# wienkers/marEx

Hardware: AMD Instinct MI355X
Metric: Mcells*timesteps/s, shifting_baseline + hobday_extreme p95 (validation+anomaly+thresholds+mask) (higher is better)
Workload: dtype f32

## Files before the change

### marex_amd/csrc/marex_tails.hip

```cpp
#include "marex_common.hip.h"
#include "marex_tails.hip.h"

typedef __amdgpu_buffer_rsrc_t tl_rsrc_t;
__device__ __forceinline__ tl_rsrc_t tl_make_rsrc(const void* base) {
    return __builtin_amdgcn_make_buffer_rsrc(const_cast<void*>(base), 0, -1, 0x00020000);
}
__device__ __forceinline__ uint4 tl_load_chunk(tl_rsrc_t r, unsigned voff, unsigned soff) {
    typedef unsigned u4 __attribute__((ext_vector_type(4)));
    const u4 v = __builtin_amdgcn_raw_buffer_load_b128(r, (int)voff, (int)soff, 0);
    return make_uint4(v.x, v.y, v.z, v.w);
}
__device__ __forceinline__ unsigned pk_sub_sat_u16(unsigned a, unsigned b) {
    unsigned r;
    asm("v_pk_sub_u16 %0, %1, %2 clamp" : "=v"(r) : "v"(a), "v"(b));
    return r;
}
__device__ __forceinline__ unsigned pk_add_u16(unsigned a, unsigned b) {
    unsigned r;
    asm("v_pk_add_u16 %0, %1, %2" : "=v"(r) : "v"(a), "v"(b));
    return r;
}
__device__ __forceinline__ unsigned pk_sub_u16(unsigned a, unsigned b) {
    unsigned r;
    asm("v_pk_sub_u16 %0, %1, %2" : "=v"(r) : "v"(a), "v"(b));
// ... 100 lines not shown
                }
                {
                    float mx = -__builtin_inff();
#pragma unroll
                    for (int u = 0; u < 16; ++u) mx = fmaxf(mx, fmaxf(va[u], vb[u]));
                    if (__builtin_amdgcn_ballot_w64(mx >= e_last) != 0) {
                        unsigned sa = ovf & 0xFFFFu, sb = ovf >> 16;
#pragma unroll
                        for (int u = 0; u < 16; ++u) {
                            if (va[u] >= e_last) sa = tail_ovf_add(sa, (unsigned)(r + u));
                            if (vb[u] >= e_last) sb = tail_ovf_add(sb, (unsigned)(r + u));
                        }
                        ovf = sa | (sb << 16);
                    }
                }
                sort16_desc(half[hb]);
            }
            unsigned v[32];
            if (short_list) {
#pragma unroll
                for (int i = 0; i < 16; ++i) {
                    v[i] = half[0][i];
                    v[16 + i] = 0u;
                }
            } else {
#pragma unroll
                for (int i = 0; i < 16; ++i) {
                    v[i] = half[0][i];
                    v[16 + i] = half[1][15 - i];
                }
                bitonic_merge_desc<32>(v);
            }
            if (active) {
#pragma unroll
                for (int j = 0; j < 4; ++j) {
                    if (j >= nch) break;
                    uint4 w0, w1;
                    unsigned* a = reinterpret_cast<unsigned*>(&w0);
                    unsigned* b = reinterpret_cast<unsigned*>(&w1);
#pragma unroll
                    for (int i = 0; i < 4; ++i) {
                        const unsigned x = v[8 * j + 2 * i], y = v[8 * j + 2 * i + 1];
                        a[i] = (x & 0xFFFFu) | (y << 16);
                        b[i] = (x >> 16) | (y & 0xFFFF0000u);
                    }
                    lists[(((size_t)d0 * NPER + p) * nch + j) * C + c] = w0;
                    lists[(((size_t)d1 * NPER + p) * nch + j) * C + c] = w1;
                }
            }
        }
        if (active) {
            aux[(size_t)d0 * C + c] = tail_aux_word(cnt & 0xFFFFu, ovf & 0xFFFFu);
            aux[(size_t)d1 * C + c] = tail_aux_word(cnt >> 16, ovf >> 16);
        }
    }
    };
    if (lean)
        body(std::true_type{});
    else
        body(std::false_type{});
}

static bool tails_geometry(int max_bucket, int list_rows, int& nper, int& nch) {
    if (max_bucket < 1 || max_bucket > TAIL_MAX_BUCKET || list_rows < 8 || list_rows > 32) return false;
    nper = (max_bucket + list_rows - 1) / list_rows;
    nch = list_rows <= 16 ? 2 : 4;
    return true;
}

extern "C" int marex_tail_lists(int max_bucket, int list_rows) {
    int nper, nch;
    return tails_geometry(max_bucket, list_rows, nper, nch) ? nper : -1;
}

int marex_tail_extract_impl(marex_ctx* ctx, const float* anom, int64_t T_out, int64_t C, const int32_t* doy_start,
                            const int32_t* doy_rows, int max_bucket, const float* edges, int nb, int list_rows, void* lists,
                            uint32_t* aux, const int* skip_chunks) {
    if (!ctx) return -1;
    if (!anom || !doy_start || !doy_rows || !edges || !lists || !aux || T_out <= 0 || C <= 0)
        return fail(ctx, -1, "marex_tail_extract_f32: null pointer or empty shape");
    if (nb < 4 || nb > TAIL_MAX_NB) return fail(ctx, -4, "marex_tail_extract_f32: nb must be in 4..%d", TAIL_MAX_NB);
    int nper, nch;
    if (!tails_geometry(max_bucket, list_rows, nper, nch))
        return fail(ctx, -4, "marex_tail_extract_f32: dayofyear buckets must hold 1..%d rows, lists 8..32 rows", TAIL_MAX_BUCKET);
    if (((uintptr_t)lists & 15) != 0) return fail(ctx, -1, "marex_tail_extract_f32: lists must be 16-byte aligned");
    if (C * 4 > 0xFFFFFFFFll) return fail(ctx, -4, "marex_tail_extract_f32: more than 2^30 cells");
    HIP_TRY(ctx, hipSetDevice(ctx->device));
    const size_t need = (size_t)T_out * sizeof(long long);
    if (need > ctx->row_off_bytes) {
        if (ctx->row_off) HIP_TRY(ctx, hipFree(ctx->row_off));
        ctx->row_off = nullptr;
        ctx->row_off_bytes = 0;
        HIP_TRY(ctx, hipMalloc((void**)&ctx->row_off, need));
        ctx->row_off_bytes = need;
    }
    const unsigned ncb = (unsigned)((C + 255) / 256);
    unsigned chunks = (2048 + ncb - 1) / ncb;
    chunks = chunks < 1 ? 1 : (chunks > 61 ? 61 : chunks);
    const size_t lds = (size_t)(nb + 1) * sizeof(float);
    {
        LaunchTimer lt(ctx, MAREX_K_TAILS);
        hipLaunchKernelGGL(k_row_offsets, dim3((unsigned)((T_out + 255) / 256)), dim3(256), 0, ctx->stream, doy_rows, (long)T_out, (long)C,
                           ctx->row_off, (int)sizeof(float));
        hipLaunchKernelGGL(k_tail_extract, dim3(ncb, chunks), dim3(256), lds, ctx->stream, anom, (long)C, doy_start, ctx->row_off, edges,
                           nb, nper, list_rows, reinterpret_cast<uint4*>(lists), aux, skip_chunks);
    }
    HIP_TRY(ctx, hipGetLastError());
    return 0;
}

extern "C" int marex_tail_extract_f32(marex_ctx* ctx, const float* anom, int64_t T_out, int64_t C, const int32_t* doy_start,
                                      const int32_t* doy_rows, int max_bucket, const float* edges, int nb, int list_rows,
                                      void* lists, uint32_t* aux) {
    return marex_tail_extract_impl(ctx, anom, T_out, C, doy_start, doy_rows, max_bucket, edges, nb, list_rows, lists, aux, nullptr);
}


#define MAREX_BUMP_KEY(u, w, ext)                                                                                   \
    "v_cmpx_lt_u32_e32 vcc, " #u ", %[n]\n\ts_cbranch_execz 1f\n\t" ext "\n\t"                                      \
    "v_subrev_u32_e32 %[t], %[b0], %[t]\n\tv_min_i32_e32 %[t], %[hi], %[t]\n\tv_and_b32_e32 %[a], -2, %[t]\n\t"       \
    "v_and_b32_e32 %[t], 1, %[t]\n\tv_lshl_add_u32 %[a], %[a], 1, %[col]\n\t"
#define MAREX_BUMP_LO(w) "v_bfe_u32 %[t], %[" #w "], 7, 9"
#define MAREX_BUMP_HI(w) "v_lshrrev_b32_e32 %[t], 23, %[" #w "]"
template <int SGN>
__device__ __forceinline__ void tl_bump_chunk(const uint4& ch, int n, int B0, int BWp1, unsigned col_lds) {
    unsigned t, a;
    unsigned long long sv;
    const int mul = SGN > 0 ? 65535 : -65535;
#define MAREX_BUMP_ADD(one) "v_mad_i32_i24 %[t], %[t], %[mul], " one "\n\tds_add_u32 %[a], %[t]\n\t"
#define MAREX_BUMP_ALL(one)                                                                                          \
    "s_mov_b64 %[sv], exec\n\t"                                                                                      \
    MAREX_BUMP_KEY(0, x, MAREX_BUMP_LO(x)) MAREX_BUMP_ADD(one) MAREX_BUMP_KEY(1, x, MAREX_BUMP_HI(x)) MAREX_BUMP_ADD(one)   \
    MAREX_BUMP_KEY(2, y, MAREX_BUMP_LO(y)) MAREX_BUMP_ADD(one) MAREX_BUMP_KEY(3, y, MAREX_BUMP_HI(y)) MAREX_BUMP_ADD(one)   \
    MAREX_BUMP_KEY(4, z, MAREX_BUMP_LO(z)) MAREX_BUMP_ADD(one) MAREX_BUMP_KEY(5, z, MAREX_BUMP_HI(z)) MAREX_BUMP_ADD(one)   \
    MAREX_BUMP_KEY(6, w, MAREX_BUMP_LO(w)) MAREX_BUMP_ADD(one) MAREX_BUMP_KEY(7, w, MAREX_BUMP_HI(w)) MAREX_BUMP_ADD(one)   \
    "1:\n\ts_mov_b64 exec, %[sv]"
    if (SGN > 0)
        asm volatile(MAREX_BUMP_ALL("1")
                     : [t] "=&v"(t), [a] "=&v"(a), [sv] "=&s"(sv)
                     : [n] "v"(n), [x] "v"(ch.x), [y] "v"(ch.y), [z] "v"(ch.z), [w] "v"(ch.w), [b0] "s"(B0), [hi] "s"(BWp1), [col] "v"(col_lds), [mul] "s"(mul)
                     : "vcc", "memory");
    else
        asm volatile(MAREX_BUMP_ALL("-1")
                     : [t] "=&v"(t), [a] "=&v"(a), [sv] "=&s"(sv)
                     : [n] "v"(n), [x] "v"(ch.x), [y] "v"(ch.y), [z] "v"(ch.z), [w] "v"(ch.w), [b0] "s"(B0), [hi] "s"(BWp1), [col] "v"(col_lds), [mul] "s"(mul)
                     : "vcc", "memory");
#undef MAREX_BUMP_ALL
#undef MAREX_BUMP_ADD
}
#undef MAREX_BUMP_KEY
#undef MAREX_BUMP_LO
#undef MAREX_BUMP_HI

#define TT_LS 34
#ifndef TT_BW
#define TT_BW 64
#endif
#define TT_MARGIN 6
#ifndef TT_STEP
#define TT_STEP 56
#endif
static_assert(TT_STEP <= TT_BW - 8, "straggler passes must overlap: a quantile bin between two tried bands would never be found");
#define TT_NPF 2

template <int NPERT>
struct TailBucket {
    uint4 c0[NPERT < TT_NPF ? NPERT : TT_NPF];
    unsigned aux;
    int d;
};

template <int P, int TC, int NT, int NPERT, int TR_ = NT / TC>
__global__ void __launch_bounds__(NT, NT == 256 ? 4 : (NT == 512 ? 2 : 1))
k_thr_tails(const uint4* __restrict__ lists, const unsigned* __restrict__ aux, int NPER, int nch, const float* __restrict__ anom,
            long C, int ny, int nx, int row0, int row1, int tiles_x, int Dd, const float* __restrict__ centres, int nb, double q,
            int wd, float lower_bound, float upper_bound, float* __restrict__ thr, marex_thr_stats* __restrict__ stats,
            unsigned long long* __restrict__ dbg, int pass_limit) {
    constexpr int TR = TR_;
    constexpr int NCELL = TR * TC;
    constexpr int NPF = NPERT < TT_NPF ? NPERT : TT_NPF;
    static_assert(NCELL <= NT && NT - NCELL < 64, "tile does not match the thread count");
    constexpr int OR = TR - 2 * P, OC = TC - 2 * P;
    __shared__ unsigned lev[NT * TT_LS];
    __shared__ unsigned tot_s[NT];
    __shared__ int s_lo[2], s_hi[2];
    __shared__ int s_iumin[2], s_iumax[2];
    __shared__ int s_est_min, s_est_max;

    const int t = threadIdx.x;
    const bool spare = NCELL < NT && t >= NCELL;
    const int tc = t % TC;
    const int tr = (TR > 1) ? (t / TC + P) % TR : 0;
    const int ci = spare ? t : tr * TC + tc;
    const int ty = (int)blockIdx.x / tiles_x, tx = (int)blockIdx.x - ty * tiles_x;
    const int jt0 = row0 + ty * OR, it0 = tx * OC;
    const int j = (ny > 0) ? jt0 - P + tr : 0;
    const int icol = it0 - P + tc;
    bool cell_valid;
    long cell;
    if (ny > 0) {
        int gi = icol % nx;
        if (gi < 0) gi += nx;
        cell_valid = (j >= 0 && j < ny) && !spare;
        cell = (long)j * nx + gi;
    } else {
        cell_valid = icol < nx && !spare;
        cell = icol < nx ? icol : nx - 1;
    }
    if (!cell_valid) cell = 0;
    const bool is_out = !spare && tr >= P && tr < TR - P && tc >= P && tc < TC - P && j < row1 && icol < nx && (ny > 0 ? j >= row0 : true);
    const int d_begin = (int)blockIdx.y * Dd;
    const int ndays = (NDOY - d_begin) < Dd ? (NDOY - d_begin) : Dd;
    const int pd = wd / 2;
    bool land = true;
    if (is_out) land = !(anom[cell] == anom[cell]);
    if (!__syncthreads_or(is_out && !land)) {
        if (is_out)
            for (int dd = 0; dd < ndays; ++dd) thr[(size_t)(d_begin + dd) * C + cell] = nan_f();
        return;
    }
    if (is_out && land)
        for (int dd = 0; dd < ndays; ++dd) thr[(size_t)(d_begin + dd) * C + cell] = nan_f();

    unsigned* mycol = &lev[ci * TT_LS];
    uint2* mycol2 = reinterpret_cast<uint2*>(mycol);
    typedef __attribute__((address_space(3))) unsigned lds_u32;
    const unsigned col_lds = (unsigned)(size_t)(lds_u32*)mycol;
    const int base_max = nb - TT_BW > 0 ? nb - TT_BW : 0;
    auto clamp_base = [&](int b) { return b < 0 ? 0 : (b > base_max ? base_max : b); };
    int B0 = 0;
    int BW = nb < TT_BW ? nb : TT_BW;
    constexpr int NLP = (TT_BW + 2 + 1) / 2;
    const unsigned voff = (unsigned)cell * 16u;
    const unsigned chunk_row = (unsigned)C * 16u;
    const size_t day_stride = (size_t)NPER * nch * (size_t)C;

    auto load_bucket = [&](int d0) {
        TailBucket<NPERT> b;
        b.d = d0;
        const tl_rsrc_t r = tl_make_rsrc(lists + (size_t)d0 * day_stride);
#pragma unroll
        for (int p = 0; p < NPF; ++p)
            b.c0[p] = (p < NPER) ? tl_load_chunk(r, voff, (unsigned)(nch * p) * chunk_row) : make_uint4(0, 0, 0, 0);
        b.aux = aux[(size_t)d0 * C + cell];
        return b;
    };
    auto bump = [&](int k, int sgn) {
        const int odd = k & 1;
        unsigned addr;
        asm("v_lshl_add_u32 %0, %1, 1, %2" : "=v"(addr) : "v"(k - odd), "v"(col_lds));
        int v;
        const int mul = sgn > 0 ? 65535 : -65535, one = sgn > 0 ? 1 : -1;
        asm("v_mad_i32_i24 %0, %1, %2, %3" : "=v"(v) : "v"(odd), "v"(mul), "v"(one));
        __hip_atomic_fetch_add((lds_u32*)(size_t)addr, (unsigned)v, __ATOMIC_RELAXED, __HIP_MEMORY_SCOPE_WORKGROUP);
    };
    int mytot = 0;
    constexpr bool ctx_asm_bump = true;
    auto bump_chunk = [&](const uint4& ch, int n, int sgn, int nfix) {
#pragma unroll
        for (int u = 0; u < 8; ++u) {
            const bool on = n > u;
            if (u >= nfix && __builtin_amdgcn_ballot_w64(on) == 0) break;
            if (on) {
                int lvl = tl_bin1(ch, u) - B0;
                lvl = lvl > BW + 1 ? BW + 1 : lvl;
                bump(lvl, sgn);
            }
        }
    };
    auto apply_bucket = [&](const TailBucket<NPERT>& b, int sgn) {
        const int cnt = cell_valid ? (int)(b.aux & 0x3FFu) : 0;
        const unsigned lim = ((unsigned)(B0 + 1) << TAIL_POS_BITS) - 1u;
        const unsigned lim_rep = lim | (lim << 16);
        const tl_rsrc_t r = tl_make_rsrc(lists + (size_t)b.d * day_stride);
        int n_in = 0;
        auto one_list = [&](const uint4& ch, int p) {
            const int n = cnt > 0 ? tl_count_above(ch, lim_rep) : 0;
            n_in += n;
            if (ctx_asm_bump) { if (sgn > 0) tl_bump_chunk<1>(ch, n, B0, BW + 1, col_lds); else tl_bump_chunk<-1>(ch, n, B0, BW + 1, col_lds); }
            else bump_chunk(ch, n, sgn, NPERT >= 3 ? 2 : 1);
            bool full = n == 8;
#pragma unroll
            for (int jj = 1; jj < 4; ++jj) {
                if (jj >= nch || __builtin_amdgcn_ballot_w64(full) == 0) break;
                const uint4 cj = tl_load_chunk(r, voff, (unsigned)(nch * p + jj) * chunk_row);
                const int nj = full ? tl_count_above(cj, lim_rep) : 0;
                n_in += nj;
                if (ctx_asm_bump) { if (sgn > 0) tl_bump_chunk<1>(cj, nj, B0, BW + 1, col_lds); else tl_bump_chunk<-1>(cj, nj, B0, BW + 1, col_lds); }
                else bump_chunk(cj, nj, sgn, 0);
                full = nj == 8;
            }
        };
#pragma unroll
        for (int p = 0; p < NPF; ++p)
            if (p < NPER) one_list(b.c0[p], p);
#pragma nounroll
        for (int p = NPF; p < NPER; p += 2) {
            const uint4 e0 = tl_load_chunk(r, voff, (unsigned)(nch * p) * chunk_row);
            const uint4 e1 = p + 1 < NPER ? tl_load_chunk(r, voff, (unsigned)(nch * (p + 1)) * chunk_row) : make_uint4(0, 0, 0, 0);
            one_list(e0, p);
            if (p + 1 < NPER) one_list(e1, p + 1);
        }
        const int below = cnt - n_in;
        if (below > 0) __hip_atomic_fetch_add((lds_u32*)(size_t)col_lds, (unsigned)(sgn > 0 ? below : -below), __ATOMIC_RELAXED,
                                              __HIP_MEMORY_SCOPE_WORKGROUP);
        mytot += sgn > 0 ? cnt : -cnt;
    };
    auto prefix = [&]() -> unsigned {
        unsigned run_rep = 0;
#pragma unroll
        for (int i = 0; i < (NLP + 1) / 2; ++i) {
            uint2 w = mycol2[i];
            w.x = pk_add_u16(w.x + (w.x << 16), run_rep);
            run_rep = __builtin_amdgcn_perm(w.x, w.x, 0x03020302u);
            w.y = pk_add_u16(w.y + (w.y << 16), run_rep);
            run_rep = __builtin_amdgcn_perm(w.y, w.y, 0x03020302u);
            mycol2[i] = w;
        }
        return run_rep & 0xFFFFu;
    };
    auto unprefix = [&]() {
        unsigned prev = 0;
#pragma unroll
        for (int i = 0; i < (NLP + 1) / 2; ++i) {
            const uint2 w = mycol2[i];
            uint2 o;
            o.x = pk_sub_u16(w.x, __builtin_amdgcn_alignbit(w.x, prev, 16));
            o.y = pk_sub_u16(w.y, __builtin_amdgcn_alignbit(w.y, w.x, 16));
            prev = w.y;
            mycol2[i] = o;
        }
    };
    auto wrap = [&](int d) { return ((d % NDOY) + NDOY) % NDOY; };
    auto rebuild = [&](int d) {
        for (int r = 0; r < TT_LS / 2; ++r) mycol2[r] = make_uint2(0u, 0u);
        mytot = 0;
        TailBucket<NPERT> cur = load_bucket(wrap(d - pd));
        for (int o = -pd + 1; o <= pd; ++o) {
            const TailBucket<NPERT> nxt = load_bucket(wrap(d + o));
            apply_bucket(cur, +1);
            cur = nxt;
        }
        apply_bucket(cur, +1);
    };
    auto pooled = [&](int k) {
        const unsigned* base = mycol + (k >> 1);
        const int sh16 = (k & 1) * 16;
        int sum = 0;
#pragma unroll
        for (int dr = -P; dr <= P; ++dr)
#pragma unroll
            for (int dc = -P; dc <= P; ++dc) sum += (int)((base[(dr * TC + dc) * TT_LS] >> sh16) & 0xFFFFu);
        return sum;
    };
    auto pooled_tot = [&]() {
        const unsigned* base = &tot_s[tr * TC + tc];
        int sum = 0;
#pragma unroll
        for (int dr = -P; dr <= P; ++dr)
#pragma unroll
            for (int dc = -P; dc <= P; ++dc) sum += (int)base[dr * TC + dc];
        return sum;
    };
    auto window = [&](int start, int (&Wv)[8]) {
        const unsigned* base = mycol + (start >> 1);
        unsigned a0 = 0, a1 = 0, a2 = 0, a3 = 0;
#pragma unroll
        for (int dr = -P; dr <= P; ++dr)
#pragma unroll
            for (int dc = -P; dc <= P; ++dc) {
                const uint2* p2 = reinterpret_cast<const uint2*>(base + (dr * TC + dc) * TT_LS);
                const uint2 u = p2[0], v = p2[1];
                a0 += u.x;
                a1 += u.y;
                a2 += v.x;
                a3 += v.y;
            }
        Wv[0] = (int)(a0 & 0xFFFFu);
        Wv[1] = (int)(a0 >> 16);
        Wv[2] = (int)(a1 & 0xFFFFu);
        Wv[3] = (int)(a1 >> 16);
        Wv[4] = (int)(a2 & 0xFFFFu);
        Wv[5] = (int)(a2 >> 16);
        Wv[6] = (int)(a3 & 0xFFFFu);
        Wv[7] = (int)(a3 >> 16);
    };
    auto find_level = [&](int hint, int khi, double qpos, int& ck, int& cb) {
        const int qf = (int)floor(qpos);
        int top = (khi - 1) & ~3;
        if (top > 60) top = 60;
        if (top < 0) top = 0;
        int start = ((hint >= 0 ? hint : (khi >> 1)) - 2) & ~3;
        start = start < 0 ? 0 : (start > top ? top : start);
        ck = 0;
        cb = 0;
        for (;;) {
            int Wv[8];
            window(start, Wv);
            const int m = (khi - start) < 8 ? (khi - start) : 8;
            int n = 0;
#pragma unroll
            for (int i = 0; i < 8; ++i) n += (i < m) && (Wv[i] <= qf);
            if (n == 0) {
                if (start == 0) {
                    ck = Wv[0];
                    return 0;
                }
                start -= 4;
                continue;
            }
            if (n == m) {
                if (m < 8 || start >= top) {
                    cb = Wv[m - 1];
                    return khi;
                }
                start += 4;
                continue;
            }
            cb = 0;
#pragma unroll
            for (int i = 0; i < 8; ++i) {
                if (i == n - 1) cb = Wv[i];
                if (i == n) ck = Wv[i];
            }
            return start + n;
        }
    };
    unsigned kmin = 0xFFFFFFFFu, kmax = 0u, nlow = 0u, nhigh = 0u;
    auto emit_threshold = [&](int d, int iu, int ck, int cb, double qpos) {
        const int il = iu > 0 ? iu - 1 : 0;
        const int cs_iu = ck;
        const int cs_il = iu > 0 ? cb : ck;
        const int diff = cs_iu - cs_il;
        const double frac = diff > 0 ? (qpos - (double)cs_il) / (double)diff : 0.5;
        const float dc = centres[iu] - centres[il];
        const double prod = frac * (double)dc;
        float t32 = (float)((double)centres[il] + prod);
        if (iu == 0) t32 = centres[0];
        const unsigned key = ordered_key(t32);
        kmin = key < kmin ? key : kmin;
        kmax = key > kmax ? key : kmax;
        if (t32 > upper_bound) ++nhigh;
        if (t32 < lower_bound) {
            ++nlow;
            t32 = lower_bound;
        }
        thr[(size_t)d * C + cell] = t32;
    };

    if (t == 0) {
        s_est_min = 0x7fffffff;
        s_est_max = -1;
        s_lo[0] = s_lo[1] = s_hi[0] = s_hi[1] = 0;
        s_iumin[0] = s_iumin[1] = 0x7fffffff;
        s_iumax[0] = s_iumax[1] = -1;
    }
    __syncthreads();
    {
        const TailBucket<NPERT> b = load_bucket(d_begin);
        const int cnt = cell_valid ? (int)(b.aux & 0x3FFu) : 0;
        if (cnt > 0) {
            int rank = (int)ceil((1.0 - q) * (double)cnt / (double)NPER);
            rank = rank < 1 ? 1 : (rank > 8 ? 8 : rank);
            unsigned key = 0;
#pragma unroll
            for (int u = 0; u < 8; ++u)
                if (u == rank - 1) key = tl_key(b.c0[0], u);
            if (key != 0u) {
                const int est = (int)(key >> TAIL_POS_BITS) - 1;
                atomicMin(&s_est_min, est);
                atomicMax(&s_est_max, est);
            }
        }
    }
    __syncthreads();
    {
        const int emin = s_est_min, emax = s_est_max;
        if (emax >= 0) {
            const int span = emax - emin + 1;
            B0 = clamp_base(span <= TT_BW - 2 * TT_MARGIN ? emin - (TT_BW - span) / 2 : emin - TT_MARGIN);
        }
    }
    BW = nb - B0 < TT_BW ? nb - B0 : TT_BW;

    int hint = -1;
    bool need_rebuild = true;
    unsigned long long n_rebuild = 0, n_pass = 0;
    TailBucket<NPERT> pin, pout;
    pin.d = pout.d = 0;
    pin.aux = pout.aux = 0;
#pragma unroll
    for (int p = 0; p < NPF; ++p) pin.c0[p] = pout.c0[p] = make_uint4(0, 0, 0, 0);
#ifdef MAREX_STAMPS
    unsigned long long st_p1 = 0, st_p2 = 0, st_bar = 0;
#define STAMP() __builtin_amdgcn_s_memtime()
#endif
    for (int dd = 0; dd < ndays; ++dd) {
        const int d = d_begin + dd;
        const int dpar = dd & 1;
#ifdef MAREX_STAMPS
        const unsigned long long tA = STAMP();
#endif
        if (need_rebuild) {
            rebuild(d);
            need_rebuild = false;
            ++n_rebuild;
            hint = -1;
        } else {
            unprefix();
            apply_bucket(pin, +1);
            apply_bucket(pout, -1);
        }
        tot_s[ci] = prefix();
        if (dd + 1 < ndays) {
            pin = load_bucket(wrap(d + 1 + pd));
            pout = load_bucket(wrap(d - pd));
        }
#ifdef MAREX_STAMPS
        const unsigned long long tB = STAMP();
        st_p1 += tB - tA;
#endif
        bool resolved = !(is_out && !land);
        int tried_lo = B0, tried_hi = B0;
        bool excursion = false;
        for (int pass = 0;; ++pass) {
            const int par = pass & 1;
#ifdef MAREX_STAMPS
            const unsigned long long tC0 = STAMP();
#endif
            __syncthreads();
#ifdef MAREX_STAMPS
            const unsigned long long tC = STAMP();
            st_bar += tC - tC0;
#endif
            if (t == 0) {
                s_lo[par ^ 1] = 0;
                s_hi[par ^ 1] = 0;
                if (pass == 0) {
                    s_iumin[dpar ^ 1] = 0x7fffffff;
                    s_iumax[dpar ^ 1] = -1;
                }
            }
            int iu_lo = 0x7fffffff, iu_hi = -1;
            if (!resolved) {
                const int tot = pooled_tot();
                if (tot > 0) {
                    const double qpos = q * (double)tot;
                    int ck, cb;
                    int k = find_level(hint, BW + 1, qpos, ck, cb);
                    int iu = -1;
                    if (k >= 1 && k <= BW) {
                        iu = B0 + k - 1;
                        hint = k;
                    } else if (k > BW && B0 + BW >= nb) {
                        iu = nb - 1;
                        k = iu - B0 + 1;
                        ck = pooled(k);
                        cb = pooled(k - 1);
                        hint = k;
                    } else if (k > BW) {
                        atomicOr(&s_hi[par], 1);
                        hint = -1;
                    } else {
                        atomicOr(&s_lo[par], 1);
                        hint = -1;
                    }
                    if (iu >= 0) {
                        emit_threshold(d, iu, ck, cb, qpos);
                        iu_lo = iu_hi = iu;
                        resolved = true;
                    }
                } else {
                    thr[(size_t)d * C + cell] = nan_f();
                    resolved = true;
                }
            }
            if (__builtin_amdgcn_ballot_w64(iu_hi >= 0) != 0) {
                const int wlo = wave_min_i32(iu_lo), whi = wave_max_i32(iu_hi);
                if ((t & 63) == 0) {
                    atomicMin(&s_iumin[dpar], wlo);
                    atomicMax(&s_iumax[dpar], whi);
                }
            }
#ifdef MAREX_STAMPS
            const unsigned long long tD = STAMP();
            st_p2 += tD - tC;
#endif
            __syncthreads();
#ifdef MAREX_STAMPS
            st_bar += STAMP() - tD;
#endif
            const int lo = s_lo[par], hi = s_hi[par];
            if (!lo && !hi) break;
            if (pass >= pass_limit) {
                if (!resolved) {
                    thr[(size_t)d * C + cell] = nan_f();
                    atomicAdd(&stats->n_unresolved, 1u);
                }
                break;
            }
            if (lo) {
                B0 = clamp_base(tried_lo - TT_STEP);
                tried_lo = B0;
            } else {
                B0 = clamp_base(tried_hi + TT_STEP);
                tried_hi = B0;
            }
            BW = nb - B0 < TT_BW ? nb - B0 : TT_BW;
            excursion = true;
            rebuild(d);
            tot_s[ci] = prefix();
            hint = -1;
            ++n_pass;
        }
        if (dd + 1 < ndays) {
            const int imin = s_iumin[dpar], imax = s_iumax[dpar];
            if (imax >= 0) {
                const int span = imax - imin + 1;
                const bool near_edge = imin - B0 < TT_MARGIN || (B0 + BW - 1) - imax < TT_MARGIN;
                if (excursion || near_edge) {
                    const int want = clamp_base(span <= TT_BW - 2 * TT_MARGIN ? imin - (TT_BW - span) / 2 : imin - TT_MARGIN);
                    if (want != B0) {
                        B0 = want;
                        BW = nb - B0 < TT_BW ? nb - B0 : TT_BW;
                        need_rebuild = true;
                    }
                }
            }
        }
    }
    for (int sft = 32; sft > 0; sft >>= 1) {
        const unsigned a = __shfl_down(kmin, sft, 64), b = __shfl_down(kmax, sft, 64);
        kmin = a < kmin ? a : kmin;
        kmax = b > kmax ? b : kmax;
        nlow += __shfl_down(nlow, sft, 64);
        nhigh += __shfl_down(nhigh, sft, 64);
    }
    if ((t & 63) == 0) {
        if (kmin != 0xFFFFFFFFu) atomicMin(&stats->min_key, kmin);
        if (kmax != 0u) atomicMax(&stats->max_key, kmax);
        if (nlow) atomicAdd(&stats->n_too_low, nlow);
        if (nhigh) atomicAdd(&stats->n_too_high, nhigh);
    }
#ifdef MAREX_STAMPS
#ifdef MAREX_STAMPS_WAVE
    const int st_wave = MAREX_STAMPS_WAVE >= 0 ? MAREX_STAMPS_WAVE : (int)((blockIdx.x + blockIdx.y) % (NT / 64));
    if (dbg && t == st_wave * 64) {
#else
    if (dbg && t == 0) {
#endif
        atomicAdd(&dbg[5], st_p1);
        atomicAdd(&dbg[6], st_p2);
        atomicAdd(&dbg[7], st_bar);
    }
#endif
    if (dbg && t == 0) {
        atomicAdd(&dbg[0], n_rebuild);
        atomicAdd(&dbg[2], n_pass);
        atomicAdd(&dbg[3], (unsigned long long)ndays);
    }
}

template <int NSC>
__global__ void __launch_bounds__(64)
k_thr_cells(const uint4* __restrict__ lists, const unsigned* __restrict__ aux, int NPER, int nch, const float* __restrict__ anom,
            long C, long c0, long c1, int nblk, const float* __restrict__ centres, int nb, double q, int wd, float lower_bound,
            float upper_bound, float* __restrict__ thr, marex_thr_stats* __restrict__ stats, unsigned long long* __restrict__ dbg) {
// ... 114 lines not shown
                        n = ne;
                        exact = true;
                        f = (double)(tot - n) <= qpos;
                        ++n_exact;
                    }
                }
                if (go) {
                    if (f) {
                        lo = mid;
                        n_lo = n;
                        lo_exact = exact;
                    } else {
                        hi = mid;
                        n_hi = n;
                    }
                }
            }
            const int iu = hi;
            if (__builtin_amdgcn_ballot_w64(iu > 0 && !lo_exact) != 0) {
                const int ne = count_exact(d, iu);
                if (iu > 0 && !lo_exact) {
                    n_lo = ne;
                    ++n_exact;
                }
            }
            const int il = iu > 0 ? iu - 1 : 0;
            const int cs_iu = tot - n_hi, cs_il = iu > 0 ? tot - n_lo : cs_iu;
            const int diff = cs_iu - cs_il;
            const double frac = diff > 0 ? (qpos - (double)cs_il) / (double)diff : 0.5;
            const float dc = centres[iu] - centres[il];
            const double prod = frac * (double)dc;
            t32 = (float)((double)centres[il] + prod);
            if (iu == 0) t32 = centres[0];
            if (valid && !land) {
                const unsigned key = ordered_key(t32);
                kmin = key < kmin ? key : kmin;
                kmax = key > kmax ? key : kmax;
                if (t32 > upper_bound) ++nhigh;
                if (t32 < lower_bound) ++nlow;
            }
            if (t32 < lower_bound) t32 = lower_bound;
        }
        if (valid) thr[(size_t)d * C + cell] = land ? nan_f() : t32;
    }
    for (int sft = 32; sft > 0; sft >>= 1) {
        const unsigned a = __shfl_down(kmin, sft, 64), b = __shfl_down(kmax, sft, 64);
        kmin = a < kmin ? a : kmin;
        kmax = b > kmax ? b : kmax;
        nlow += __shfl_down(nlow, sft, 64);
        nhigh += __shfl_down(nhigh, sft, 64);
        n_exact += __shfl_down(n_exact, sft, 64);
    }
    if (lane == 0) {
        if (kmin != 0xFFFFFFFFu) atomicMin(&stats->min_key, kmin);
        if (kmax != 0u) atomicMax(&stats->max_key, kmax);
        if (nlow) atomicAdd(&stats->n_too_low, nlow);
        if (nhigh) atomicAdd(&stats->n_too_high, nhigh);
        if (dbg && n_exact) atomicAdd(&dbg[1], n_exact);
    }
}

extern "C" int marex_hobday_thresholds_tails_f32(marex_ctx* ctx, const void* lists, const uint32_t* aux, int list_rows,
                                                 const float* anom, int64_t T_out, int64_t C, int ny, int nx, int max_bucket,
                                                 const float* centres,
                                                 int nb, double q, int wd, int ws, float lower_bound, float upper_bound, int row0,
                                                 int row1, float* thr_doy_major, marex_thr_stats* stats) {
    if (!ctx) return -1;
    if (!lists || !aux || !anom || !centres || !thr_doy_major || !stats || T_out <= 0 || C <= 0)
        return fail(ctx, -1, "marex_hobday_thresholds_tails_f32: null pointer or empty shape");
    if (wd < 3 || wd > 365 || (wd & 1) == 0)
        return fail(ctx, -1, "marex_hobday_thresholds_tails_f32: window_days_hobday must be odd and in 3..365");
    if (ws < 1 || (ws & 1) == 0) return fail(ctx, -1, "marex_hobday_thresholds_tails_f32: window_spatial_hobday must be odd");
    if (!(q > 0.0 && q <= 1.0)) return fail(ctx, -1, "marex_hobday_thresholds_tails_f32: q must be in (0, 1]");
    if (ny == 0) {
        if (ws > 1) return fail(ctx, -1, "marex_hobday_thresholds_tails_f32: spatial pooling needs a structured grid");
        nx = (int)C;
        row0 = 0;
        row1 = 1;
    } else if ((int64_t)ny * nx != C) {
        return fail(ctx, -1, "marex_hobday_thresholds_tails_f32: ny*nx != C");
    } else if (row0 < 0 || row1 > ny || row0 >= row1) {
        return fail(ctx, -1, "marex_hobday_thresholds_tails_f32: need 0 <= row0 < row1 <= ny");
    }
    const int p = ws / 2;
    if (nb < 4 || nb > TAIL_MAX_NB || max_bucket < 1 || max_bucket > TAIL_MAX_BUCKET || p > 3 ||
        (int64_t)max_bucket * wd * ws * ws > 65535 || C > (1 << 24))
        return fail(ctx, -4, "marex_hobday_thresholds_tails_f32: shape outside the tail kernel (nb <= %d, buckets <= %d rows, "
                             "ws <= 7, pooled window <= 65535 samples)", TAIL_MAX_NB, TAIL_MAX_BUCKET);
    HIP_TRY(ctx, hipSetDevice(ctx->device));
    int NPER, nch;
    if (!tails_geometry(max_bucket, list_rows, NPER, nch))
        return fail(ctx, -4, "marex_hobday_thresholds_tails_f32: %d rows per bucket in lists of %d", max_bucket, list_rows);
    const int cells_opt = ctx_opt(ctx, "THR_CELLS", 1);
    if (p == 0 && cells_opt && (cells_opt == 2 ? wd * NPER <= 128 : wd * NPER <= 16)) {
        const long c0 = ny > 0 ? (long)row0 * nx : 0, c1 = ny > 0 ? (long)row1 * nx : (long)C;
        const long ncg = (c1 - c0 + 63) / 64;
        int nblk = (int)((32L * 4 * device_cus(ctx) + ncg - 1) / ncg);
        nblk = nblk < 1 ? 1 : (nblk > 12 ? 12 : nblk);
        nblk = ctx_opt(ctx, "THR_CELLS_BLOCKS", nblk);
        LaunchTimer lt(ctx, MAREX_K_THRESHOLDS);
        const size_t lds = (size_t)((wd * NPER + 3) & ~3) * 64 * sizeof(uint4);
        const int nslot = (wd * NPER + 3) & ~3;
        const bool cached = nslot == 12 && ctx_opt(ctx, "THR_CELLS_CACHE", 1);
        if (lds > 64 * 1024) HIP_TRY(ctx, hipFuncSetAttribute((const void*)k_thr_cells<0>, hipFuncAttributeMaxDynamicSharedMemorySize, (int)lds));
        hipLaunchKernelGGL(cached ? k_thr_cells<12> : k_thr_cells<0>, dim3((unsigned)ncg, (unsigned)nblk), dim3(64), lds, ctx->stream,
                           reinterpret_cast<const uint4*>(lists), aux, NPER, nch, anom, (long)C, c0, c1, nblk, centres, nb, q, wd,
                           lower_bound, upper_bound, thr_doy_major, stats, ctx_debug_counters(ctx));
        HIP_TRY(ctx, hipGetLastError());
        return 0;
    }
    if (NPER > 6)
        return fail(ctx, -4, "marex_hobday_thresholds_tails_f32: %d rows per bucket in lists of %d: more than 6 lists", max_bucket, list_rows);
    const int tile_pref = ctx_opt(ctx, "THR_TILE", (ny > 0 && p > 0 && max_bucket >= 24) ? 32 : 16);
    const bool half = (ny > 0 && p == 2) && tile_pref == 3216 && (row1 - row0) >= 12 && nx >= 16;
    const bool big = !half && (ny > 0 && p > 0) && tile_pref == 32 && (row1 - row0) >= 16 && nx >= 16;
    const int NT = big ? 1024 : (half ? 512 : 256);
    int TR = (ny > 0 && p > 0) ? (big ? 32 : 16) : 1, TC = NT / TR;
    const size_t lds_pad = (size_t)ctx_opt(ctx, "THR_LDS_PAD", 0) * 1024;
    bool tall = false;
    if (big && p == 2 && ctx_opt(ctx, "THR_TALL", 1)) {
        auto ntiles = [&](int tr, int tc) {
            return (long)((nx + tc - 2 * p - 1) / (tc - 2 * p)) * ((row1 - row0 + tr - 2 * p - 1) / (tr - 2 * p));
        };
        tall = ntiles(34, 30) < ntiles(32, 32) && (row1 - row0) >= 30;
        if (tall) TR = 34, TC = 30;
    }
    const int OR = TR - 2 * p, OC = TC - 2 * p;
    const int tiles_x = (nx + OC - 1) / OC, tiles_y = (row1 - row0 + OR - 1) / OR;
    int Dd = ctx_opt(ctx, "THR_DD", 0);
    if (Dd < 1 || Dd > NDOY) {
        const long cus = device_cus(ctx), tiles = (long)tiles_x * tiles_y;
        const long slots = cus * (big ? 1 : (half ? 2 : 4));
        long best = -1;
        for (int d = 16; d <= NDOY; ++d) {
            const long blocks = tiles * ((NDOY + d - 1) / d);
            const long cost = ((blocks + slots - 1) / slots) * (d + wd);
            if (best < 0 || cost < best) best = cost, Dd = d;
        }
    }
    dim3 grid((unsigned)(tiles_x * tiles_y), (unsigned)((NDOY + Dd - 1) / Dd));
    unsigned long long* dbg = ctx_debug_counters(ctx);
    const uint4* tl = reinterpret_cast<const uint4*>(lists);
    const int pass_limit = ctx_opt(ctx, "THR_PASS_LIMIT", 2 * (nb / TT_STEP) + 9);
#define MAREX_TT_ARGS tl, aux, NPER, nch, anom, (long)C, ny, nx, row0, row1, tiles_x, Dd, centres, nb, q, wd, lower_bound, upper_bound, thr_doy_major, stats, dbg, pass_limit
#define MAREX_TT_LAUNCH(PP, TCC, NTT, ...)                                                                                           \
    do {                                                                                                                             \
        if (NPER <= 1)                                                                                                               \
            hipLaunchKernelGGL((k_thr_tails<PP, TCC, NTT, 1, ##__VA_ARGS__>), grid, dim3(NTT), lds_pad, ctx->stream, MAREX_TT_ARGS); \
        else if (NPER <= 2)                                                                                                          \
            hipLaunchKernelGGL((k_thr_tails<PP, TCC, NTT, 2, ##__VA_ARGS__>), grid, dim3(NTT), lds_pad, ctx->stream, MAREX_TT_ARGS); \
        else                                                  \
            hipLaunchKernelGGL((k_thr_tails<PP, TCC, NTT, 3, ##__VA_ARGS__>), grid, dim3(NTT), lds_pad, ctx->stream, MAREX_TT_ARGS); \
    } while (0)
    {
        LaunchTimer lt(ctx, MAREX_K_THRESHOLDS);
        if (TR == 1)
            MAREX_TT_LAUNCH(0, 256, 256);
        else if (half)
            MAREX_TT_LAUNCH(2, 32, 512, 16);
        else if (big && p == 1)
            MAREX_TT_LAUNCH(1, 32, 1024);
        else if (big && p == 2 && tall)
            MAREX_TT_LAUNCH(2, 30, 1024, 34);
        else if (big && p == 2)
            MAREX_TT_LAUNCH(2, 32, 1024);
        else if (big)
            MAREX_TT_LAUNCH(3, 32, 1024);
        else if (p == 1)
            MAREX_TT_LAUNCH(1, 16, 256);
        else if (p == 2)
            MAREX_TT_LAUNCH(2, 16, 256);
        else
            MAREX_TT_LAUNCH(3, 16, 256);
    }
#undef MAREX_TT_LAUNCH
#undef MAREX_TT_ARGS
    HIP_TRY(ctx, hipGetLastError());
    return 0;
}

#ifndef MASK_WAVES
#define MASK_WAVES 5
#endif
template <int NPERT>
__global__ void __launch_bounds__(256, MASK_WAVES)
k_mask_tails(const uint4* __restrict__ lists, const unsigned* __restrict__ aux, int NPER_all, int nch, const float* __restrict__ anom,
             const float* __restrict__ edges, int nb, const float* __restrict__ thr, const int* __restrict__ doy_start,
             const int* __restrict__ doy_rows, const long long* __restrict__ row_off, const long long* __restrict__ row_off_anom,
             long C, long c0, long c1, unsigned char* __restrict__ out, unsigned long long* __restrict__ n_true,
             unsigned long long* __restrict__ dbg) {
    const int nchunk = (int)gridDim.y;
    const int dA = (int)blockIdx.y * NDOY / nchunk, dB = ((int)blockIdx.y + 1) * NDOY / nchunk;
    const long c = (c0 & ~255L) + ((long)blockIdx.x * 256 + threadIdx.x) * 4;
    unsigned cnt_true = 0;
    unsigned long long n_slow = 0;
    if (c >= c0 && c < c1) {
        const float inv_width = (float)(nb - 1) / (edges[nb] - edges[1]);
        for (int d = dA; d < dB; ++d) {
            const int r0 = doy_start[d], nd = doy_start[d + 1] - r0;
            if (nd == 0) continue;
            const float4 th4 = *reinterpret_cast<const float4*>(thr + (size_t)d * C + c);
            const float tv[4] = {th4.x, th4.y, th4.z, th4.w};
            const uint4 ax = *reinterpret_cast<const uint4*>(aux + (size_t)d * C + c);
            const unsigned av[4] = {ax.x, ax.y, ax.z, ax.w};
            unsigned beyond = 0;
            unsigned bits[4][4];
            unsigned lim_ge[4];
            int kt[4];
            bool slow = false, walk[4];
#pragma unroll
            for (int i = 0; i < 4; ++i) {
                bits[i][0] = bits[i][1] = bits[i][2] = bits[i][3] = 0u;
                const bool isnum = tv[i] == tv[i];
                kt[i] = isnum ? digitize_bin(tv[i], edges, nb, inv_width) : nb;
                slow = slow || (isnum && (av[i] & TAIL_AUX_BEYOND) && ((av[i] & TAIL_AUX_MANY) || kt[i] >= nb));
                beyond |= (isnum && (av[i] & TAIL_AUX_BEYOND)) ? 1u : 0u;
                walk[i] = isnum && (av[i] & 0x3FFu) > 0 && kt[i] < nb;
                const unsigned lim = ((unsigned)(kt[i] + 1) << TAIL_POS_BITS) - 1u;
                lim_ge[i] = lim | (lim << 16);
            }
            auto set_prefix = [&](const uint4& q, int n, int i) {
#pragma unroll
                for (int u = 0; u < 8; ++u) {
                    const bool on = n > u;
                    if (u >= 1 && __builtin_amdgcn_ballot_w64(on) == 0) break;
                    if (on) {
                        const int pos = (int)(tl_key(q, u) & (TAIL_MAX_BUCKET - 1));
#pragma unroll
                        for (int wi = 0; wi < 4; ++wi)
                            if ((pos >> 5) == wi) bits[i][wi] |= 1u << (pos & 31);
                    }
                }
            };
            if (__builtin_amdgcn_ballot_w64(!slow) != 0)
            for (int pg = 0; pg < NPER_all; pg += NPERT) {
                const int NPER = (NPER_all - pg) < NPERT ? (NPER_all - pg) : NPERT;
                uint4 ch[NPERT][4];
                const uint4* row0 = lists + (((size_t)d * NPER_all + pg) * nch) * C + c;
#pragma unroll
                for (int p = 0; p < NPERT; ++p)
#pragma unroll
                    for (int i = 0; i < 4; ++i) ch[p][i] = p < NPER ? row0[(size_t)(p * nch) * C + i] : make_uint4(0, 0, 0, 0);
            float cand_val[NPERT][4];
            int cand_pos[NPERT][4];
            unsigned redo = 0;
            {
#pragma unroll
                for (int p = 0; p < NPERT; ++p) {
#pragma unroll
                    for (int i = 0; i < 4; ++i) {
                        cand_pos[p][i] = -1;
                        cand_val[p][i] = 0.f;
                        if (p < NPER && walk[i] && !slow) {
                            const unsigned lgt = lim_ge[i] + (0x10001u << TAIL_POS_BITS);
                            const int n_ge = tl_count_above(ch[p][i], lim_ge[i]);
                            const int n_gt = tl_count_above(ch[p][i], lgt);
                            set_prefix(ch[p][i], n_gt, i);
                            if (n_ge == 8 || n_ge - n_gt > 1) redo |= 1u << (p * 4 + i);
                            if (n_ge - n_gt == 1) {
                                const unsigned w[4] = {ch[p][i].x, ch[p][i].y, ch[p][i].z, ch[p][i].w};
                                unsigned lo = w[0], hi = w[1];
#pragma unroll
                                for (int k = 1; k < 4; ++k)
                                    if ((n_gt >> 1) == k) lo = w[k], hi = k < 3 ? w[k + 1] : 0u;
                                const unsigned key = (n_gt & 1) ? (lo >> 16) : (lo & 0xFFFFu);
                                (void)hi;
                                cand_pos[p][i] = (int)(key & (TAIL_MAX_BUCKET - 1));
                            }
                        }
                    }
                }
#pragma unroll
                for (int p = 0; p < NPERT; ++p)
#pragma unroll
                    for (int i = 0; i < 4; ++i)
                        if (cand_pos[p][i] >= 0)
                            cand_val[p][i] = *reinterpret_cast<const float*>(reinterpret_cast<const char*>(anom) + row_off_anom[r0 + cand_pos[p][i]] + (size_t)(c + i) * 4);
#pragma unroll
                for (int p = 0; p < NPERT; ++p)
#pragma unroll
                    for (int i = 0; i < 4; ++i)
                        if (cand_pos[p][i] >= 0 && cand_val[p][i] >= tv[i]) {
                            const int pos = cand_pos[p][i];
#pragma unroll
                            for (int wi = 0; wi < 4; ++wi)
                                if ((pos >> 5) == wi) bits[i][wi] |= 1u << (pos & 31);
                        }
                if (__builtin_amdgcn_ballot_w64(redo != 0u) != 0) {
#pragma unroll
                    for (int p = 0; p < NPERT; ++p)
#pragma unroll
                        for (int i = 0; i < 4; ++i) {
                            if (__builtin_amdgcn_ballot_w64((redo >> (p * 4 + i)) & 1u) == 0) continue;
                            bool on = (redo >> (p * 4 + i)) & 1u;
                            for (int jj = 0; jj < nch; ++jj) {
                                if (__builtin_amdgcn_ballot_w64(on) == 0) break;
                                const uint4 q = on ? row0[(size_t)(p * nch + jj) * C + i] : make_uint4(0, 0, 0, 0);
#pragma unroll
                                for (int u = 0; u < 8; ++u) {
                                    const unsigned key = tl_key(q, u);
                                    const int bin = (int)(key >> TAIL_POS_BITS) - 1, pos = (int)(key & (TAIL_MAX_BUCKET - 1));
                                    on = on && bin >= kt[i];
                                    if (on) {
                                        bool ext = bin > kt[i];
                                        if (!ext) ext = *reinterpret_cast<const float*>(reinterpret_cast<const char*>(anom) + row_off_anom[r0 + pos] + (size_t)(c + i) * 4) >= tv[i];
                                        if (ext) {
#pragma unroll
                                            for (int wi = 0; wi < 4; ++wi)
                                                if ((pos >> 5) == wi) bits[i][wi] |= 1u << (pos & 31);
// ... 133 lines not shown
```

Before: 309,700.

## Add lean tail-threshold kernel specialization with fused inline-asm list scan

Adds a compile-time specialized 'lean' variant of the thresholds kernel for the common geometry (six lists, two chunks each, big tiles, p=2). It fixes NPER and nch as template constants, replaces per-list count-then-bump with a single inline-asm scan that compares, bumps LDS counters and propagates a 'full' wave mask in one pass, and walks day pointers incrementally instead of recomputing wrapped offsets. The goal is to cut VALU instructions, ballots and address arithmetic in the per-day sliding-window update. The cost is extra template instantiations and hand-written asm that only fires on this exact geometry, selected through an option that defaults to on.

```diff
diff --git a/marex_amd/csrc/marex_tails.hip b/marex_amd/csrc/marex_tails.hip
--- a/marex_amd/csrc/marex_tails.hip
+++ b/marex_amd/csrc/marex_tails.hip
@@ -276,6 +276,46 @@
 #undef MAREX_BUMP_LO
 #undef MAREX_BUMP_HI
 
+#define MAREX_SCAN_KEY(ext)                                                                                           \
+    ext "\n\tv_cmpx_lt_u32_e32 vcc, %[b0], %[t]\n\ts_cbranch_execz 1f\n\t"
+#define MAREX_SCAN_ADD(one)                                                                                           \
+    "v_subrev_u32_e32 %[t], %[b0], %[t]\n\tv_min_i32_e32 %[t], %[hi], %[t]\n\tv_and_b32_e32 %[a], -2, %[t]\n\t"         \
+    "v_and_b32_e32 %[t], 1, %[t]\n\tv_lshl_add_u32 %[a], %[a], 1, %[col]\n\tv_mad_i32_i24 %[t], %[t], %[mul], " one "\n\t" \
+    "ds_add_u32 %[a], %[t]\n\tv_add_u32_e32 %[n], 1, %[n]\n\t"
+#define MAREX_SCAN_LO(w) "v_bfe_u32 %[t], %[" #w "], 7, 9"
+#define MAREX_SCAN_HI(w) "v_lshrrev_b32_e32 %[t], 23, %[" #w "]"
+template <int SGN>
+__device__ __forceinline__ unsigned long long tl_scan_chunk(const uint4& ch, unsigned long long pm, int& n, int B0, int BWp1,
+                                                            unsigned col_lds) {
+    unsigned t, a;
+    unsigned long long sv, full;
+    const int mul = SGN > 0 ? 65535 : -65535;
+#define MAREX_SCAN_ALL(one)                                                                                           \
+    "s_mov_b64 %[sv], exec\n\ts_mov_b64 %[full], 0\n\ts_and_b64 exec, exec, %[pm]\n\ts_cbranch_execz 1f\n\t"          \
+    MAREX_SCAN_KEY(MAREX_SCAN_LO(x)) MAREX_SCAN_ADD(one) MAREX_SCAN_KEY(MAREX_SCAN_HI(x)) MAREX_SCAN_ADD(one)         \
+    MAREX_SCAN_KEY(MAREX_SCAN_LO(y)) MAREX_SCAN_ADD(one) MAREX_SCAN_KEY(MAREX_SCAN_HI(y)) MAREX_SCAN_ADD(one)         \
+    MAREX_SCAN_KEY(MAREX_SCAN_LO(z)) MAREX_SCAN_ADD(one) MAREX_SCAN_KEY(MAREX_SCAN_HI(z)) MAREX_SCAN_ADD(one)         \
+    MAREX_SCAN_KEY(MAREX_SCAN_LO(w)) MAREX_SCAN_ADD(one) MAREX_SCAN_KEY(MAREX_SCAN_HI(w))                             \
+    "s_mov_b64 %[full], exec\n\t" MAREX_SCAN_ADD(one)                                                                \
+    "1:\n\ts_mov_b64 exec, %[sv]"
+    if (SGN > 0)
+        asm volatile(MAREX_SCAN_ALL("1")
+                     : [t] "=&v"(t), [a] "=&v"(a), [sv] "=&s"(sv), [full] "=&s"(full), [n] "+v"(n)
+                     : [pm] "s"(pm), [x] "v"(ch.x), [y] "v"(ch.y), [z] "v"(ch.z), [w] "v"(ch.w), [b0] "s"(B0), [hi] "s"(BWp1), [col] "v"(col_lds), [mul] "s"(mul)
+                     : "vcc", "memory");
+    else
+        asm volatile(MAREX_SCAN_ALL("-1")
+                     : [t] "=&v"(t), [a] "=&v"(a), [sv] "=&s"(sv), [full] "=&s"(full), [n] "+v"(n)
+                     : [pm] "s"(pm), [x] "v"(ch.x), [y] "v"(ch.y), [z] "v"(ch.z), [w] "v"(ch.w), [b0] "s"(B0), [hi] "s"(BWp1), [col] "v"(col_lds), [mul] "s"(mul)
+                     : "vcc", "memory");
+#undef MAREX_SCAN_ALL
+    return full;
+}
+#undef MAREX_SCAN_KEY
+#undef MAREX_SCAN_ADD
+#undef MAREX_SCAN_LO
+#undef MAREX_SCAN_HI
+
 #define TT_LS 34
 #ifndef TT_BW
 #define TT_BW 64
@@ -292,17 +332,21 @@
     uint4 c0[NPERT < TT_NPF ? NPERT : TT_NPF];
     unsigned aux;
     int d;
+    const uint4* base;
 };
 
-template <int P, int TC, int NT, int NPERT, int TR_ = NT / TC>
+template <int P, int TC, int NT, int NPERT, int TR_ = NT / TC, int LN = 0, int LC = 0>
 __global__ void __launch_bounds__(NT, NT == 256 ? 4 : (NT == 512 ? 2 : 1))
-k_thr_tails(const uint4* __restrict__ lists, const unsigned* __restrict__ aux, int NPER, int nch, const float* __restrict__ anom,
+k_thr_tails(const uint4* __restrict__ lists, const unsigned* __restrict__ aux, int NPER_rt, int nch_rt, const float* __restrict__ anom,
             long C, int ny, int nx, int row0, int row1, int tiles_x, int Dd, const float* __restrict__ centres, int nb, double q,
             int wd, float lower_bound, float upper_bound, float* __restrict__ thr, marex_thr_stats* __restrict__ stats,
             unsigned long long* __restrict__ dbg, int pass_limit) {
     constexpr int TR = TR_;
     constexpr int NCELL = TR * TC;
     constexpr int NPF = NPERT < TT_NPF ? NPERT : TT_NPF;
+    constexpr bool LEAN = LN > 0;
+    static_assert(!LEAN || (LN >= NPF && LN <= 2 * NPERT && LC >= 2 && LC <= 4), "lean list geometry");
+    const int NPER = LEAN ? LN : NPER_rt, nch = LEAN ? LC : nch_rt;
     static_assert(NCELL <= NT && NT - NCELL < 64, "tile does not match the thread count");
     constexpr int OR = TR - 2 * P, OC = TC - 2 * P;
     __shared__ unsigned lev[NT * TT_LS];
@@ -367,6 +411,17 @@
         for (int p = 0; p < NPF; ++p)
             b.c0[p] = (p < NPER) ? tl_load_chunk(r, voff, (unsigned)(nch * p) * chunk_row) : make_uint4(0, 0, 0, 0);
         b.aux = aux[(size_t)d0 * C + cell];
+        b.base = lists + (size_t)d0 * day_stride;
+        return b;
+    };
+    auto load_bucket_at = [&](const uint4* lbase, const unsigned* abase) {
+        TailBucket<NPERT> b;
+        b.d = 0;
+        b.base = lbase;
+        const tl_rsrc_t r = tl_make_rsrc(lbase);
+#pragma unroll
+        for (int p = 0; p < NPF; ++p) b.c0[p] = tl_load_chunk(r, voff, (unsigned)(nch * p) * chunk_row);
+        b.aux = abase[cell];
         return b;
     };
     auto bump = [&](int k, int sgn) {
@@ -396,7 +451,7 @@
         const int cnt = cell_valid ? (int)(b.aux & 0x3FFu) : 0;
         const unsigned lim = ((unsigned)(B0 + 1) << TAIL_POS_BITS) - 1u;
         const unsigned lim_rep = lim | (lim << 16);
-        const tl_rsrc_t r = tl_make_rsrc(lists + (size_t)b.d * day_stride);
+        const tl_rsrc_t r = tl_make_rsrc(LEAN ? b.base : lists + (size_t)b.d * day_stride);
         int n_in = 0;
         auto one_list = [&](const uint4& ch, int p) {
             const int n = cnt > 0 ? tl_count_above(ch, lim_rep) : 0;
@@ -415,18 +470,31 @@
                 full = nj == 8;
             }
         };
+        const unsigned long long live = LEAN ? __builtin_amdgcn_ballot_w64(cnt > 0) : 0ull;
+        auto scan_list = [&](const uint4& ch, int p) {
+            unsigned long long f = sgn > 0 ? tl_scan_chunk<1>(ch, live, n_in, B0, BW + 1, col_lds) : tl_scan_chunk<-1>(ch, live, n_in, B0, BW + 1, col_lds);
+#pragma unroll
+            for (int jj = 1; jj < LC; ++jj) {
+                if (f == 0) break;
+                const uint4 cj = tl_load_chunk(r, voff, (unsigned)(nch * p + jj) * chunk_row);
+                f = sgn > 0 ? tl_scan_chunk<1>(cj, f, n_in, B0, BW + 1, col_lds) : tl_scan_chunk<-1>(cj, f, n_in, B0, BW + 1, col_lds);
+            }
+        };
+        auto a_list = [&](const uint4& ch, int p) {
+            if (LEAN) scan_list(ch, p); else one_list(ch, p);
+        };
 #pragma unroll
         for (int p = 0; p < NPF; ++p)
-            if (p < NPER) one_list(b.c0[p], p);
+            if (p < NPER) a_list(b.c0[p], p);
 #pragma nounroll
         for (int p = NPF; p < NPER; p += 2) {
             const uint4 e0 = tl_load_chunk(r, voff, (unsigned)(nch * p) * chunk_row);
             const uint4 e1 = p + 1 < NPER ? tl_load_chunk(r, voff, (unsigned)(nch * (p + 1)) * chunk_row) : make_uint4(0, 0, 0, 0);
-            one_list(e0, p);
-            if (p + 1 < NPER) one_list(e1, p + 1);
+            a_list(e0, p);
+            if (p + 1 < NPER) a_list(e1, p + 1);
         }
         const int below = cnt - n_in;
-        if (below > 0) __hip_atomic_fetch_add((lds_u32*)(size_t)col_lds, (unsigned)(sgn > 0 ? below : -below), __ATOMIC_RELAXED,
+        if (LEAN || below > 0) __hip_atomic_fetch_add((lds_u32*)(size_t)col_lds, (unsigned)(sgn > 0 ? below : -below), __ATOMIC_RELAXED,
                                               __HIP_MEMORY_SCOPE_WORKGROUP);
         mytot += sgn > 0 ? cnt : -cnt;
     };
@@ -613,6 +681,12 @@
     TailBucket<NPERT> pin, pout;
     pin.d = pout.d = 0;
     pin.aux = pout.aux = 0;
+    pin.base = pout.base = lists;
+    int in_d = wrap(d_begin + pd), out_d = wrap(d_begin - pd - 1);
+    const uint4* in_l = lists + (size_t)in_d * day_stride;
+    const uint4* out_l = lists + (size_t)out_d * day_stride;
+    const unsigned* in_a = aux + (size_t)in_d * C;
+    const unsigned* out_a = aux + (size_t)out_d * C;
 #pragma unroll
     for (int p = 0; p < NPF; ++p) pin.c0[p] = pout.c0[p] = make_uint4(0, 0, 0, 0);
 #ifdef MAREX_STAMPS
@@ -636,7 +710,18 @@
             apply_bucket(pout, -1);
         }
         tot_s[ci] = prefix();
-        if (dd + 1 < ndays) {
+        if (LEAN) {
+            in_d = in_d + 1 == NDOY ? 0 : in_d + 1;
+            in_l = in_d == 0 ? lists : in_l + day_stride;
+            in_a = in_d == 0 ? aux : in_a + C;
+            out_d = out_d + 1 == NDOY ? 0 : out_d + 1;
+            out_l = out_d == 0 ? lists : out_l + day_stride;
+            out_a = out_d == 0 ? aux : out_a + C;
+            if (dd + 1 < ndays) {
+                pin = load_bucket_at(in_l, in_a);
+                pout = load_bucket_at(out_l, out_a);
+            }
+        } else if (dd + 1 < ndays) {
             pin = load_bucket(wrap(d + 1 + pd));
             pout = load_bucket(wrap(d - pd));
         }
@@ -1057,9 +1142,14 @@
         else                                                  \
             hipLaunchKernelGGL((k_thr_tails<PP, TCC, NTT, 3, ##__VA_ARGS__>), grid, dim3(NTT), lds_pad, ctx->stream, MAREX_TT_ARGS); \
     } while (0)
+    const bool lean = NPER == 6 && nch == 2 && big && p == 2 && ctx_opt(ctx, "THR_LEAN", 1) != 0;
     {
         LaunchTimer lt(ctx, MAREX_K_THRESHOLDS);
-        if (TR == 1)
+        if (lean && tall)
+            hipLaunchKernelGGL((k_thr_tails<2, 30, 1024, 3, 34, 6, 2>), grid, dim3(1024), lds_pad, ctx->stream, MAREX_TT_ARGS);
+        else if (lean)
+            hipLaunchKernelGGL((k_thr_tails<2, 32, 1024, 3, 32, 6, 2>), grid, dim3(1024), lds_pad, ctx->stream, MAREX_TT_ARGS);
+        else if (TR == 1)
             MAREX_TT_LAUNCH(0, 256, 256);
         else if (half)
             MAREX_TT_LAUNCH(2, 32, 512, 16);
```

Result: faster. 318,100, median of 6 (+2.7%).
